# BAMresearch/PGDrome

Measured on AMD Instinct MI355X. Metric: PGD fixed-point iters/sec + SpMV HBM GB/s, 256^3 P1 space x 1D param, higher is better.
Workload: dtype f64

## Files before the change

include/pgd_amd.h:

```cpp
#ifndef PGD_AMD_H
#define PGD_AMD_H

#include <stdint.h>

#ifdef __cplusplus
extern "C" {
#endif

typedef int64_t pgd_handle;

enum {
    PGD_OK = 0,
    PGD_ERR_INVALID = -1,
    PGD_ERR_HIP = -2,
    PGD_ERR_NOMEM = -3,
    PGD_ERR_LIMIT = -4,
    PGD_ERR_SINGULAR = -5,
    PGD_ERR_NODEVICE = -6,
    PGD_ERR_TIMEOUT = -7,
    PGD_ERR_PEER = -8
};

enum {
    PGD_ATOM_MASS = 0,
// ... 9 lines not shown
};

int pgd_ctx_create(int device, void *stream, pgd_handle *ctx);
int pgd_ctx_destroy(pgd_handle ctx);
int pgd_sync(pgd_handle ctx);
const char *pgd_last_error(pgd_handle ctx);
int pgd_version(void);
int pgd_device_count(void);

int pgd_mesh_upload(pgd_handle ctx, const double *coords, int64_t nv, int gdim,
                    const int32_t *cells, int64_t nc, int nvpc, pgd_handle *mesh);
int pgd_mesh_blocked(pgd_handle ctx, pgd_handle scalar_mesh, int ncomp, pgd_handle *mesh);
int pgd_mesh_info(pgd_handle ctx, pgd_handle mesh, int64_t *nv, int64_t *nc, int64_t *nnz,
                  int32_t *max_row_len, int32_t *kl, int32_t *ku);
int pgd_mesh_pattern_download(pgd_handle ctx, pgd_handle mesh, int32_t *row_ptr, int32_t *cols);
int pgd_mesh_dict_count(pgd_handle ctx, pgd_handle mesh, int32_t *count);
int pgd_mesh_sym_info(pgd_handle ctx, pgd_handle mesh, int32_t *slots, int32_t *nx, int32_t *ny);
int pgd_mesh_lattice(pgd_handle ctx, pgd_handle mesh, int32_t *is_lattice, double *steps);
int pgd_mesh_free(pgd_handle ctx, pgd_handle mesh);

int pgd_vec_alloc(pgd_handle ctx, int64_t n, pgd_handle *vec);
int pgd_vec_free(pgd_handle ctx, pgd_handle vec);
int pgd_vec_size(pgd_handle ctx, pgd_handle vec, int64_t *n);
int pgd_vec_upload(pgd_handle ctx, pgd_handle vec, const double *host, int64_t offset, int64_t count);
int pgd_vec_download(pgd_handle ctx, pgd_handle vec, double *host, int64_t offset, int64_t count);
int pgd_vec_ptr(pgd_handle ctx, pgd_handle vec, void **device_ptr);
int pgd_vec_fill(pgd_handle ctx, pgd_handle vec, double value);
int pgd_vec_copy(pgd_handle ctx, pgd_handle dst, pgd_handle src);
int pgd_vec_scale(pgd_handle ctx, pgd_handle vec, double a);
int pgd_vec_mul(pgd_handle ctx, pgd_handle y, pgd_handle a, pgd_handle x);
int pgd_vec_axpy(pgd_handle ctx, pgd_handle y, double a, pgd_handle x);
int pgd_vec_set(pgd_handle ctx, pgd_handle vec, const int32_t *idx, const double *val, int64_t n);
int pgd_vec_lincomb(pgd_handle ctx, pgd_handle y, const pgd_handle *xs, const double *coefs, int k);
int pgd_vec_dot(pgd_handle ctx, pgd_handle x, pgd_handle y, int64_t lo, int64_t hi, double *out);

int pgd_atom_assemble(pgd_handle ctx, pgd_handle mesh, int kind, int da, int db,
                      pgd_handle wvec, pgd_handle *atom);
int pgd_atom_assemble_cells(pgd_handle ctx, pgd_handle mesh, int kind, int da, int db, pgd_handle wvec,
                            const uint8_t *cell_mask, int64_t nc, pgd_handle *atom);
int pgd_atom_assemble_cellwise(pgd_handle ctx, pgd_handle mesh, int kind, int da, int db, pgd_handle wvec,
                               pgd_handle cvec, const uint8_t *cell_mask, int64_t nc, pgd_handle *atom);
int pgd_atom_assemble_facets(pgd_handle ctx, pgd_handle mesh, const int32_t *facets, int64_t nf, int nvpf,
                             pgd_handle *atom);
int pgd_atom_embed(pgd_handle ctx, pgd_handle blocked_mesh, pgd_handle src, int cv, int cu, double coef,
                   pgd_handle dst, pgd_handle *out);
int pgd_atom_upload(pgd_handle ctx, pgd_handle mesh, const double *vals, pgd_handle *atom);
int pgd_atom_download(pgd_handle ctx, pgd_handle atom, double *vals);
int pgd_atom_free(pgd_handle ctx, pgd_handle atom);

int pgd_op_combine(pgd_handle ctx, pgd_handle mesh, const pgd_handle *atoms, const double *coefs,
                   int n, const int32_t *bc_dofs, int64_t nbc, pgd_handle *op);

int pgd_spmv(pgd_handle ctx, pgd_handle A, pgd_handle x, pgd_handle y, int64_t r0, int64_t r1);
int pgd_bilinear(pgd_handle ctx, pgd_handle A, pgd_handle x, pgd_handle y, int64_t r0, int64_t r1,
                 double *out);
int pgd_bilinear_many(pgd_handle ctx, pgd_handle A, pgd_handle x, const pgd_handle *ys, int ny,
                      int64_t r0, int64_t r1, double *out);

int pgd_pcg_solve(pgd_handle ctx, pgd_handle op, pgd_handle b, pgd_handle x, double rtol,
                  double atol, int maxit, int *iters, double *relres);
int pgd_band_solve(pgd_handle ctx, pgd_handle op, pgd_handle b, pgd_handle x);

#define PGD_NSLOTS 64
int pgd_slots_ptr(pgd_handle ctx, void **device_ptr);
int pgd_slots_download(pgd_handle ctx, double *out, int first, int count);
int pgd_slots_upload(pgd_handle ctx, const double *in, int first, int count);
// ... 39 lines not shown
                  int64_t hi_ghost);
int pgd_comm_allreduce_slots(pgd_handle ctx, int first_slot, int count);

#define PGD_PUSH_BLOB_BYTES 256
int pgd_comm_push_export(pgd_handle ctx, int64_t n, int64_t own0, int64_t own1, int64_t lo_ghost, int64_t hi_ghost,
                         uint8_t *blob );
int pgd_comm_push_attach(pgd_handle ctx, const uint8_t *lower_blob, const uint8_t *upper_blob, int *state);
int pgd_comm_push(pgd_handle ctx, int mode, int *state);
int pgd_comm_allreduce_attach(pgd_handle ctx, const uint8_t *all_blobs, int *state);
int pgd_comm_allreduce_direct(pgd_handle ctx, int mode, int *state);
int pgd_pcg_solve_sharded(pgd_handle ctx, pgd_handle A, pgd_handle b, pgd_handle x, int64_t own0,
                          int64_t own1, int64_t lo_ghost, int64_t hi_ghost, double rtol, double atol,
                          int maxit, int *iters, double *rel_res);

int pgd_bicgstab_solve(pgd_handle ctx, pgd_handle A, pgd_handle b, pgd_handle x, double rtol, double atol,
                       int maxit, int *iters, double *rel_res);

int pgd_start_gram(pgd_handle ctx, pgd_handle A, const pgd_handle *vecs, int k, pgd_handle b, int64_t r0,
                   int64_t r1, double *out);
int pgd_start_residual(pgd_handle ctx, pgd_handle A, int k, const double *coefs, pgd_handle b, pgd_handle r);

int pgd_vec_multidot(pgd_handle ctx, pgd_handle x, const pgd_handle *ys, int k, int64_t lo, int64_t hi,
                     double *out);

int pgd_vec_multidot_pair(pgd_handle ctx, pgd_handle x0, pgd_handle x1, const pgd_handle *ys, int k, int64_t lo,
                          int64_t hi, double *out);

enum { PGD_EVAL_STATS = 1, PGD_EVAL_ENVELOPE = 2, PGD_EVAL_EXCEED = 4, PGD_EVAL_FIELDS = 8 };
int pgd_eval_batch(pgd_handle ctx, const pgd_handle *modes, int k, const double *coefs, int64_t s, int want,
                   double threshold, double *sample_stats, pgd_handle env_min, pgd_handle env_max, pgd_handle exceed,
                   pgd_handle fields);

enum {
    PGD_TUNE_PCG_RECOMPUTE_Q = 53,
    PGD_TUNE_EVAL_SAMPLE_CHUNK = 52,
    PGD_TUNE_EVAL_GRID_MAX = 51,
    PGD_TUNE_EVAL_VARIANT = 50,
    PGD_TUNE_PUSH_IN_UPDATE = 49,
    PGD_TUNE_STENCIL_ROWS = 48,
    PGD_TUNE_DIA_MARCH3 = 47,
    PGD_TUNE_SHARD_ONE_MARCH = 46,
    PGD_TUNE_HALO_OVERLAP_MIN_ROWS = 45,
    PGD_TUNE_COMM_SELF_PERIODIC = 44,
    PGD_TUNE_PCG_DERIVE_SCALED = 43,
    PGD_TUNE_MG_MARCH_MIN = 42,
    PGD_TUNE_MG_CHUNK = 41,
    PGD_TUNE_PCG_PRECOND = 40,
    PGD_TUNE_CLS_CACHE = 39,
    PGD_TUNE_STENCIL_DEPTH = 38,
    PGD_TUNE_STENCIL_WG_PER_CU = 37,
    PGD_TUNE_SPMV_ZCHUNK_STENCIL = 36,
    PGD_TUNE_SPMV_STENCIL = 35,
    PGD_TUNE_FAULT_STALL_MS = 34,
    PGD_TUNE_FAULT_STAGE = 33,
    PGD_TUNE_SPMV_ZCHUNK_CODED2 = 32,
    PGD_TUNE_PCG_PIPELINE = 31,
    PGD_TUNE_PCG_EXACT_PHASE = 30,
    PGD_TUNE_PCG_FOLD_FINISH = 29,
    PGD_TUNE_LAZY_CSR = 28,
    PGD_TUNE_ATOM_FAST = 27,
    PGD_TUNE_SPMV_ROWS = 1,
    PGD_TUNE_SPMV_GRID_MIN_BYTES = 8,
    PGD_TUNE_PCG_FOLD_REDUCE = 12,
    PGD_TUNE_PCG_SCALED = 10,
    PGD_TUNE_SPMV_ZCHUNK_FORCE = 7,
    PGD_TUNE_PCG_SMALL_ROWS = 26,
// ... 49 lines not shown
```

pgdrome_amd/_lib.py:

```python
from __future__ import annotations

import ctypes as C
from pathlib import Path

import numpy as np

LIB_PATH = Path(__file__).resolve().parent / "lib" / "libpgd_amd.so"

H = C.c_int64
I64 = C.c_int64
I32 = C.c_int32
F64 = C.c_double
PD = C.POINTER(C.c_double)
PI32 = C.POINTER(C.c_int32)
PI64 = C.POINTER(C.c_int64)
PH = C.POINTER(C.c_int64)
VP = C.c_void_p

PU8 = C.POINTER(C.c_uint8)
HALO_FN = C.CFUNCTYPE(C.c_int, VP, H, I64, I64, I64, I64)
ALLREDUCE_FN = C.CFUNCTYPE(C.c_int, VP, C.c_int, C.c_int)

SIGNATURES = {
    "pgd_ctx_create": (C.c_int, [C.c_int, VP, PH]),
    "pgd_ctx_destroy": (C.c_int, [H]),
    "pgd_sync": (C.c_int, [H]),
    "pgd_last_error": (C.c_char_p, [H]),
    "pgd_version": (C.c_int, []),
    "pgd_device_count": (C.c_int, []),
    "pgd_mesh_upload": (C.c_int, [H, PD, I64, C.c_int, PI32, I64, C.c_int, PH]),
    "pgd_mesh_blocked": (C.c_int, [H, H, C.c_int, PH]),
    "pgd_atom_embed": (C.c_int, [H, H, H, C.c_int, C.c_int, F64, H, PH]),
    "pgd_mesh_info": (C.c_int, [H, H, PI64, PI64, PI64, PI32, PI32, PI32]),
    "pgd_mesh_pattern_download": (C.c_int, [H, H, PI32, PI32]),
    "pgd_mesh_sym_info": (C.c_int, [H, H, PI32, PI32, PI32]),
    "pgd_mesh_dict_count": (C.c_int, [H, H, PI32]),
    "pgd_mesh_lattice": (C.c_int, [H, H, PI32, PD]),
    "pgd_mesh_free": (C.c_int, [H, H]),
    "pgd_vec_alloc": (C.c_int, [H, I64, PH]),
    "pgd_vec_free": (C.c_int, [H, H]),
    "pgd_vec_size": (C.c_int, [H, H, PI64]),
    "pgd_vec_upload": (C.c_int, [H, H, PD, I64, I64]),
    "pgd_vec_download": (C.c_int, [H, H, PD, I64, I64]),
    "pgd_vec_ptr": (C.c_int, [H, H, C.POINTER(VP)]),
    "pgd_vec_fill": (C.c_int, [H, H, F64]),
    "pgd_vec_copy": (C.c_int, [H, H, H]),
    "pgd_vec_scale": (C.c_int, [H, H, F64]),
    "pgd_vec_mul": (C.c_int, [H, H, H, H]),
    "pgd_vec_axpy": (C.c_int, [H, H, F64, H]),
    "pgd_vec_set": (C.c_int, [H, H, PI32, PD, I64]),
    "pgd_vec_lincomb": (C.c_int, [H, H, PH, PD, C.c_int]),
    "pgd_vec_dot": (C.c_int, [H, H, H, I64, I64, PD]),
    "pgd_eval_batch": (C.c_int, [H, PH, C.c_int, PD, I64, C.c_int, F64, PD, H, H, H, H]),
    "pgd_atom_assemble": (C.c_int, [H, H, C.c_int, C.c_int, C.c_int, H, PH]),
    "pgd_atom_assemble_cells": (C.c_int, [H, H, C.c_int, C.c_int, C.c_int, H, PU8, I64, PH]),
    "pgd_atom_assemble_cellwise": (C.c_int, [H, H, C.c_int, C.c_int, C.c_int, H, H, PU8, I64, PH]),
    "pgd_atom_assemble_facets": (C.c_int, [H, H, PI32, I64, C.c_int, PH]),
    "pgd_atom_upload": (C.c_int, [H, H, PD, PH]),
    "pgd_atom_download": (C.c_int, [H, H, PD]),
    "pgd_atom_free": (C.c_int, [H, H]),
    "pgd_op_combine": (C.c_int, [H, H, PH, PD, C.c_int, PI32, I64, PH]),
    "pgd_spmv": (C.c_int, [H, H, H, H, I64, I64]),
    "pgd_bilinear": (C.c_int, [H, H, H, H, I64, I64, PD]),
    "pgd_bilinear_many": (C.c_int, [H, H, H, PH, C.c_int, I64, I64, PD]),
    "pgd_start_gram": (C.c_int, [H, H, PH, C.c_int, H, I64, I64, PD]),
    "pgd_start_residual": (C.c_int, [H, H, C.c_int, PD, H, H]),
    "pgd_mg_slab_setup": (C.c_int, [H, H, C.c_int, C.c_int, I64, I64, C.POINTER(I64), C.POINTER(C.c_int)]),
    "pgd_mg_slab_fix_start": (C.c_int, [H, H, H, H, I64, I64]),
    "pgd_mg_slab_down": (C.c_int, [H, H, H]),
    "pgd_mg_slab_restrict": (C.c_int, [H, H, H]),
    "pgd_mg_coarse": (C.c_int, [H, H, H]),
    "pgd_mg_slab_up": (C.c_int, [H, H, H, H, H, C.c_int, PD]),
    "pgd_bicgstab_solve": (C.c_int, [H, H, H, H, C.c_double, C.c_double, C.c_int, C.POINTER(C.c_int), PD]),
    "pgd_atom_product_form": (C.c_int, [H, H, C.POINTER(C.c_int)]),
    "pgd_vec_multidot": (C.c_int, [H, H, PH, C.c_int, I64, I64, PD]),
    "pgd_vec_multidot_pair": (C.c_int, [H, H, H, PH, C.c_int, I64, I64, PD]),
    "pgd_pcg_solve": (C.c_int, [H, H, H, H, F64, F64, C.c_int, C.POINTER(C.c_int), PD]),
    "pgd_band_solve": (C.c_int, [H, H, H, H]),
    "pgd_slots_ptr": (C.c_int, [H, C.POINTER(VP)]),
    "pgd_slots_download": (C.c_int, [H, PD, C.c_int, C.c_int]),
    "pgd_slots_upload": (C.c_int, [H, PD, C.c_int, C.c_int]),
    "pgd_flags_reset": (C.c_int, [H]),
    "pgd_flags_download": (C.c_int, [H, PI32, PI32, PI32]),
    "pgd_op_diag_inv": (C.c_int, [H, H, H]),
# ... 216 lines not shown
    def vec_download(self, v, offset=0, count=None):
        if count is None:
            count = self.vec_size(v) - offset
        out = np.empty(count, dtype=np.float64)
        self._ck(self.lib.pgd_vec_download(self.h, v, dptr(out), int(offset), int(count)))
        return out

    def vec_ptr(self, v):
        p = VP()
        self._ck(self.lib.pgd_vec_ptr(self.h, v, C.byref(p)))
        return p.value

    def vec_fill(self, v, a):
        self._ck(self.lib.pgd_vec_fill(self.h, v, float(a)))

    def vec_copy(self, dst, src):
        self._ck(self.lib.pgd_vec_copy(self.h, dst, src))

    def vec_scale(self, v, a):
        self._ck(self.lib.pgd_vec_scale(self.h, v, float(a)))

    def vec_mul(self, y, a, x):
        self._ck(self.lib.pgd_vec_mul(self.h, y, a, x))

    def vec_axpy(self, y, a, x):
        self._ck(self.lib.pgd_vec_axpy(self.h, y, float(a), x))

    def vec_lincomb(self, y, xs, coefs):
        k = len(xs)
        arr = (H * max(k, 1))(*[int(x) for x in xs])
        cf = np.ascontiguousarray(coefs, dtype=np.float64)
        self._ck(self.lib.pgd_vec_lincomb(self.h, y, arr, dptr(cf) if k else None, k))

    def eval_batch(self, modes, coefs, stats=True, env_min=0, env_max=0, exceed=0, threshold=0.0, fields=0):
        k = len(modes)
        cf = np.ascontiguousarray(coefs, dtype=np.float64)
        if cf.ndim != 2 or cf.shape[0] != k:
            raise ValueError("eval_batch: coefs must have shape (len(modes), samples), got %r for %d modes" % (cf.shape, k))
        s = cf.shape[1]
        want = (EVAL_STATS if stats else 0) | (EVAL_ENVELOPE if (env_min or env_max) else 0) | \
               (EVAL_EXCEED if exceed else 0) | (EVAL_FIELDS if fields else 0)
        arr = (H * max(k, 1))(*[int(x) for x in modes])
        out = np.empty((3, s), dtype=np.float64) if stats else None
        self._ck(self.lib.pgd_eval_batch(self.h, arr, k, dptr(cf) if cf.size else None, s, want, float(threshold),
                                         dptr(out) if stats else None, int(env_min), int(env_max), int(exceed), int(fields)))
        return out

    def vec_set(self, v, idx, val):
        idx = np.ascontiguousarray(idx, dtype=np.int32)
        val = np.ascontiguousarray(np.broadcast_to(np.asarray(val, dtype=np.float64), idx.shape))
        self._ck(self.lib.pgd_vec_set(self.h, v, iptr(idx), dptr(val), idx.size))

    def vec_dot(self, x, y, lo=0, hi=-1):
        out = F64()
        self._ck(self.lib.pgd_vec_dot(self.h, x, y, int(lo), int(hi), C.byref(out)))
        return out.value

    def vec_multidot(self, x, ys, lo=0, hi=-1):
        k = len(ys)
        arr = (H * k)(*[int(v) for v in ys])
        out = np.zeros(k, dtype=np.float64)
        self._ck(self.lib.pgd_vec_multidot(self.h, x, arr, k, int(lo), int(hi), dptr(out)))
        return out

    def vec_multidot_pair(self, x0, x1, ys, lo=0, hi=-1):
        k = len(ys)
# ... 395 lines not shown
```

pgdrome_amd/csrc/pgd_internal.h:

```cpp
#pragma once

#include <hip/hip_runtime.h>

#include <cstdint>
#include <cstdio>
#include <map>
#include <memory>
#include <string>
#include <vector>

#include "../../include/pgd_amd.h"

namespace pgd {

constexpr int WAVE = 64;
constexpr int TPB = 256;
constexpr int MAX_VEC_BLOCKS = 2048;
constexpr int N_XCD = 8;
constexpr int DICT_MAXP = 256;
constexpr int DICT_DLEN = 32;
constexpr size_t PAD_BYTES = 256;

enum { S_PQ = 2, S_TOL2 = 5, S_DMIN = 7 , S_TMP = 8  };
enum { S1_RZ = 24, S1_RR = 25, S1_ALPHA = 26, S1_BETA = 27, S1_PQ = 28, S1_QQ = 29,
// ... 161 lines not shown
    int *flags = nullptr;
    double *partials = nullptr;
    int64_t partials_cap = 0;
    int64_t partials_off = 0;
    double *work[7] = {nullptr, nullptr, nullptr, nullptr, nullptr, nullptr, nullptr};
    int64_t work_cap[7] = {0, 0, 0, 0, 0, 0, 0};
    uint8_t *mask = nullptr;
    int64_t mask_cap = 0;
    int *ibuf = nullptr;
    int64_t ibuf_cap = 0;
    std::vector<int32_t> set_idx_host;
    std::vector<double> set_val_host;
    int *set_idx = nullptr;
    double *set_vals = nullptr;
    int64_t set_idx_cap = 0, set_vals_cap = 0;
    int32_t set_idx_max = 0;
    bool set_idx_on_dev = false, set_val_on_dev = false;

    Comm comm;

    int num_cu = 256;
    int spmv_dict = 1;
    int spmv_rows = 64;
    int64_t spmv_grid_min_plane_bytes = 0;
    int spmv_zchunk_force = 0;
    int fault_iteration = -1;
    int fault_stage = 0;
    int fault_stall_ms = 0;
    int64_t pcg_small_ss_rows = (int64_t)1 << 22;
    int pcg_small_ss = 1;
    int pcg_stream_hints = 1;
    int pcg_lag_x = 1;
    int pcg_recompute_q = 1;
    int64_t pcg_recompute_launches = 0;
    int asm_lattice = 1;
    int spmv_fetch_depth = 6;
    int spmv_zchunk_coded2 = 96;
    int spmv_zchunk_coded = 24;
    int pcg_exact_phase = 1;
    int pcg_fold_finish = 1;
    int atom_fast = 1;
    int lazy_csr = 1;
    uint64_t next_serial = 1;
    int pcg_precond = 0;
    struct Mg *mg = nullptr;
    struct Mg *mg_slab = nullptr;
    int64_t mg_solves = 0, mg_fallbacks = 0;
    struct Vmg *vmg = nullptr;
    int64_t vmg_solves = 0, vmg_fallbacks = 0, vmg_marches = 0;
    double vmg_setup_ms = 0.0;
    struct Cmg *cmg = nullptr;
    int64_t cmg_solves = 0, cmg_fallbacks = 0, cmg_marches = 0;
    double cmg_setup_ms = 0.0;
    int eval_variant = 1, eval_grid_max = 0, eval_chunk = 0;
    double *eval_pin = nullptr;
    size_t eval_pin_bytes = 0;
    hipEvent_t eval_ev[2] = {nullptr, nullptr};
    bool eval_ev_set[2] = {false, false};
    int mg_chunk = 2;
    int mg_march_min = 64;
    int cls_cache_on = 1;
    int64_t cls_fast = 0, cls_full = 0;
    int spmv_stencil = 1;
    int spmv_zchunk_stencil = 0;
    int stencil_depth = 0;
    int stencil_wg_per_cu = 2;
// ... 213 lines not shown
```

pgdrome_amd/csrc/pgd_spmv.hip:

```cpp
#include <chrono>
#include <cstring>

#include "pgd_internal.h"
#include "pgd_dia_march.h"

#include <algorithm>

namespace pgd {

constexpr int SPMV_CAP = 4096;
constexpr int SPMV_VROUNDS = 8;
constexpr int SPMV_CROUNDS = 4;
constexpr int MAXY = 8;

struct SpmvArgs {
    const int *row_ptr, *cols;
    const double *vals, *x, *w;
    double *y, *partials;
    const int *flags;
    int row_begin, row_end;
};

typedef double d2_t __attribute__((ext_vector_type(2)));
typedef int i4_t __attribute__((ext_vector_type(4)));
// ... 2347 lines not shown
}

constexpr int GRAM_MAXV = 17;
struct MultiDotArgs {
    const double *w, *b;
    const double *v[GRAM_MAXV];
    int nv;
    int64_t lo, hi;
    double *partials;
};

__global__ __launch_bounds__(TPB) void k_multidot(MultiDotArgs A) {
    __shared__ double s_red[4];
    double acc[GRAM_MAXV + 1];
#pragma unroll
    for (int m = 0; m <= GRAM_MAXV; ++m) acc[m] = 0.0;
    for (int64_t i = A.lo + (int64_t)blockIdx.x * TPB + threadIdx.x; i < A.hi; i += (int64_t)gridDim.x * TPB) {
        const double wi = A.w[i];
        double last = 0.0;
#pragma unroll
        for (int m = 0; m < GRAM_MAXV; ++m)
            if (m < A.nv) { last = A.v[m][i]; acc[m] = fma(last, wi, acc[m]); }
        acc[GRAM_MAXV] = fma(last, A.b[i], acc[GRAM_MAXV]);
    }
#pragma unroll
    for (int m = 0; m <= GRAM_MAXV; ++m) {
        if (m < A.nv || m == GRAM_MAXV) {
            const double sum = block_sum(acc[m], s_red);
            if (threadIdx.x == 0) A.partials[(int64_t)blockIdx.x * (A.nv + 1) + (m == GRAM_MAXV ? A.nv : m)] = sum;
        }
    }
}

constexpr int PAIR_MAXV = 16;
struct MultiDot2Args {
    const double *w0, *w1;
    const double *v[PAIR_MAXV];
    int nv;
    int64_t lo, hi;
    double *partials;
};

__global__ __launch_bounds__(TPB) void k_multidot2(MultiDot2Args A) {
    __shared__ double s_red[4];
    double a0[PAIR_MAXV], a1[PAIR_MAXV];
#pragma unroll
    for (int m = 0; m < PAIR_MAXV; ++m) a0[m] = a1[m] = 0.0;
    for (int64_t i = A.lo + (int64_t)blockIdx.x * TPB + threadIdx.x; i < A.hi; i += (int64_t)gridDim.x * TPB) {
        const double x0 = A.w0[i], x1 = A.w1[i];
#pragma unroll
        for (int m = 0; m < PAIR_MAXV; ++m)
            if (m < A.nv) { const double y = A.v[m][i]; a0[m] = fma(y, x0, a0[m]); a1[m] = fma(y, x1, a1[m]); }
    }
#pragma unroll
    for (int m = 0; m < PAIR_MAXV; ++m) {
        if (m < A.nv) {
            const double s0 = block_sum(a0[m], s_red);
            const double s1 = block_sum(a1[m], s_red);
            if (threadIdx.x == 0) {
                A.partials[(int64_t)blockIdx.x * (2 * A.nv) + m] = s0;
                A.partials[(int64_t)blockIdx.x * (2 * A.nv) + A.nv + m] = s1;
            }
        }
    }
}

// ... 125 lines not shown
    if (knob == PGD_TUNE_STENCIL_WG_PER_CU && value >= 1 && value <= 8) { c->stencil_wg_per_cu = (int)value; return PGD_OK; }
    if (knob == PGD_TUNE_FAULT_STAGE && value >= 0 && value <= 4) { c->fault_stage = (int)value; return PGD_OK; }
    if (knob == PGD_TUNE_FAULT_STALL_MS && value >= 0 && value <= 20000) { c->fault_stall_ms = (int)value; return PGD_OK; }
    if (knob == PGD_TUNE_COMBINE_DIA && value >= 0 && value <= 1) { c->spmv_combine_dia = (int)value; return PGD_OK; }
    if (knob == PGD_TUNE_SPMV_VARIANT && value >= 0 && value <= 2) { c->spmv_variant = (int)value; return PGD_OK; }
    if (knob == PGD_TUNE_SPMV_ROW_CLASSES && value >= 0 && value <= 1) { c->spmv_classes = (int)value; return PGD_OK; }
    if (knob == PGD_TUNE_ASM_LATTICE && value >= 0 && value <= 3) { c->asm_lattice = (int)value; return PGD_OK; }
    if (knob == PGD_TUNE_PCG_LAG_X && value >= 0 && value <= 1) { c->pcg_lag_x = (int)value; return PGD_OK; }
    if (knob == PGD_TUNE_PCG_STREAM_HINTS && value >= 0 && value <= 1) { c->pcg_stream_hints = (int)value; return PGD_OK; }
    if (knob == PGD_TUNE_PCG_SMALL_SINGLE_SYNC && value >= 0 && value <= 1) { c->pcg_small_ss = (int)value; return PGD_OK; }
    if (knob == PGD_TUNE_PCG_SMALL_ROWS && value >= 0) { c->pcg_small_ss_rows = value; return PGD_OK; }
    if (knob == PGD_TUNE_SPMV_FETCH_DEPTH && (value == 3 || value == 6)) { c->spmv_fetch_depth = (int)value; return PGD_OK; }
    if (knob == PGD_TUNE_SPMV_ZCHUNK_CODED2 && value >= 0 && value <= 1020) { c->spmv_zchunk_coded2 = (int)value / 6 * 6; return PGD_OK; }
    if (knob == PGD_TUNE_PCG_PIPELINE && value >= 0 && value <= 1) { c->pcg_pipeline = (int)value; return PGD_OK; }
    if (knob == PGD_TUNE_PCG_EXACT_PHASE && value >= 0 && value <= 1) { c->pcg_exact_phase = (int)value; return PGD_OK; }
    if (knob == PGD_TUNE_PCG_FOLD_FINISH && value >= 0 && value <= 1) { c->pcg_fold_finish = (int)value; return PGD_OK; }
    if (knob == PGD_TUNE_ATOM_FAST && value >= 0 && value <= 1) { c->atom_fast = (int)value; return PGD_OK; }
    if (knob == PGD_TUNE_LAZY_CSR && value >= 0 && value <= 1) { c->lazy_csr = (int)value; return PGD_OK; }
    if (knob == PGD_TUNE_SPMV_ZCHUNK_CODED && value >= 3 && value <= 1024) { c->spmv_zchunk_coded = (int)value; return PGD_OK; }
    if (knob == PGD_TUNE_PCG_PRECOND && value >= 0 && value <= 3) { c->pcg_precond = (int)value; return PGD_OK; }
    if (knob == PGD_TUNE_PCG_DERIVE_SCALED && value >= 0 && value <= 1) { c->pcg_derive_scaled = (int)value; return PGD_OK; }
    if (knob == PGD_TUNE_COMM_SELF_PERIODIC && value >= 0 && value <= 1) { c->comm.self_periodic = value != 0; return PGD_OK; }
    if (knob == PGD_TUNE_HALO_OVERLAP_MIN_ROWS && value >= 0) { c->comm.overlap_min_rows = value; return PGD_OK; }
    if (knob == PGD_TUNE_SHARD_ONE_MARCH && value >= 0 && value <= 1) { c->shard_one_march = (int)value; return PGD_OK; }
    if (knob == PGD_TUNE_DIA_MARCH3 && value >= 0 && value <= 1) { c->dia_march3 = (int)value; return PGD_OK; }
    if (knob == PGD_TUNE_STENCIL_ROWS && (value == 0 || value == 2 || value == 4)) { c->stencil_rows = (int)value; return PGD_OK; }
    if (knob == PGD_TUNE_PUSH_IN_UPDATE && (value == 0 || value == 1)) { c->push_in_update = (int)value; return PGD_OK; }
    if (knob == PGD_TUNE_MG_CHUNK && value >= 2 && value <= 16 && value % 2 == 0) { c->mg_chunk = (int)value; return PGD_OK; }
    if (knob == PGD_TUNE_MG_MARCH_MIN && value >= 0 && value <= 1 << 20) { c->mg_march_min = (int)value; return PGD_OK; }
    if (knob == PGD_TUNE_EVAL_VARIANT && value >= 0 && value <= 1) { c->eval_variant = (int)value; return PGD_OK; }
    if (knob == PGD_TUNE_EVAL_GRID_MAX && value >= 0 && value <= 1 << 20) { c->eval_grid_max = (int)value; return PGD_OK; }
    if (knob == PGD_TUNE_EVAL_SAMPLE_CHUNK && value >= 0 && value <= 1024) { c->eval_chunk = (int)value; return PGD_OK; }
    if (knob == PGD_TUNE_PCG_RECOMPUTE_Q && value >= 0 && value <= 1) { c->pcg_recompute_q = (int)value; return PGD_OK; }
    return fail(c, PGD_ERR_INVALID, "tune: unknown knob %d or value out of range", knob);
}

int pgd_spmv(pgd_handle h, pgd_handle ah, pgd_handle xh, pgd_handle yh, int64_t r0, int64_t r1) {
    PGD_CTX(c, h);
    Csr *a = get_csr(c, ah);
    Mesh *m = a ? get_mesh(c, a->mesh) : nullptr;
    Vec *x = get_vec(c, xh), *y = get_vec(c, yh);
    if (!a || !m || !x || !y || x->n != m->nv || y->n != m->nv || x == y)
        return fail(c, PGD_ERR_INVALID, "spmv: invalid handles, size mismatch or x aliases y");
    if (atom_fast_form(c, m, a, r0, r1)) return launch_spmv_op(c, m, a, x->d, y->d, nullptr, r0, r1, false, true, nullptr, nullptr);
    if (c->spmv_sym && c->atom_fast && m->sym_nx > 0 && !a->immutable && a->uvals && a->uvals_valid && !a->uvals_scaled && !a->st_virtual) {
        const int64_t plane = (int64_t)m->sym_nx * m->sym_ny;
        const int64_t q0 = r0 < 0 ? 0 : r0, q1 = r1 < 0 ? m->nv : r1;
        if (q0 >= 0 && q1 <= m->nv && q0 <= q1 && q0 % plane == 0 && q1 % plane == 0)
            return launch_spmv_op(c, m, a, x->d, y->d, nullptr, q0, q1, false, true, nullptr, nullptr);
    }
    PGD_TRY(ensure_vals(c, m, a));
    return launch_spmv(c, m, a->vals, x->d, y->d, nullptr, r0, r1, false, true, nullptr, nullptr);
}

int pgd_bilinear(pgd_handle h, pgd_handle ah, pgd_handle xh, pgd_handle yh, int64_t r0, int64_t r1, double *out) {
    PGD_CTX(c, h);
    Csr *a = get_csr(c, ah);
    Mesh *m = a ? get_mesh(c, a->mesh) : nullptr;
    Vec *x = get_vec(c, xh), *y = get_vec(c, yh);
    if (!a || !m || !x || !y || !out || x->n != m->nv || y->n != m->nv)
        return fail(c, PGD_ERR_INVALID, "bilinear: invalid handles or size mismatch");
    int nparts = 0;
    PGD_TRY(ensure_vals(c, m, a));
    PGD_TRY(launch_spmv(c, m, a->vals, y->d, nullptr, x->d, r0, r1, true, false, nullptr, &nparts));
    if (nparts == 0) { *out = 0.0; return PGD_OK; }
    PGD_TRY(reduce_partials(c, c->partials, nparts, 1, S_TMP, -1, 0, 0));
// ... 58 lines not shown
    Csr *a = get_csr(c, ah);
    Mesh *m = a ? get_mesh(c, a->mesh) : nullptr;
    Vec *x = get_vec(c, xh), *y = get_vec(c, yh), *w = get_vec(c, wh);
    if (!a || !m || !x || !y || !w || x->n != m->nv || y->n != m->nv || w->n != m->nv || x == y ||
        slot < 0 || slot >= PGD_NSLOTS)
        return fail(c, PGD_ERR_INVALID, "spmv_dot_slot: invalid handles, sizes or slot");
    int nparts = 0;
    PGD_TRY(launch_spmv_op(c, m, a, x->d, y->d, w->d, r0, r1, true, true, c->flags, &nparts));
    if (nparts == 0) {
        PGD_HIP(c, hipMemsetAsync(c->slots + slot, 0, sizeof(double), c->stream));
        return PGD_OK;
    }
    return reduce_partials(c, c->partials, nparts, 1, slot, 0, 0, 0);
}

int pgd_vec_multidot(pgd_handle h, pgd_handle xh, const pgd_handle *yhs, int k, int64_t lo, int64_t hi, double *out) {
    PGD_CTX(c, h);
    Vec *x = get_vec(c, xh);
    if (!x || !yhs || !out || k < 1 || k > 256) return fail(c, PGD_ERR_INVALID, "vec_multidot: invalid handles or count (1..256)");
    if (hi < 0) hi = x->n;
    if (lo < 0 || lo > hi || hi > x->n) return fail(c, PGD_ERR_INVALID, "vec_multidot: bad range");
    std::vector<const double *> y((size_t)k);
    for (int j = 0; j < k; ++j) {
        Vec *v = get_vec(c, yhs[j]);
        if (!v || v->n != x->n) return fail(c, PGD_ERR_INVALID, "vec_multidot: invalid vector %d", j);
        y[(size_t)j] = v->d;
    }
    for (int j = 0; j < k; ++j) out[j] = 0.0;
    if (hi == lo) return PGD_OK;
    PGD_TRY(ensure_work(c, 6, 2 * (int64_t)MAX_VEC_BLOCKS > 512 ? 2 * (int64_t)MAX_VEC_BLOCKS : 512));
    double *res = c->work[6];
    const int g = grid_for(hi - lo);
    PGD_TRY(ensure_partials(c, (int64_t)g * (GRAM_MAXV + 1) > 4 * MAX_VEC_BLOCKS ? (int64_t)g * (GRAM_MAXV + 1) : 4 * MAX_VEC_BLOCKS));
    int off = 0;
    for (int j0 = 0; j0 < k; j0 += GRAM_MAXV) {
        const int nv = std::min(GRAM_MAXV, k - j0);
        MultiDotArgs A;
        A.w = x->d; A.b = x->d; A.nv = nv; A.lo = lo; A.hi = hi; A.partials = c->partials;
        for (int q = 0; q < GRAM_MAXV; ++q) A.v[q] = y[(size_t)(j0 + std::min(q, nv - 1))];
        k_multidot<<<g, TPB, 0, c->stream>>>(A);
        PGD_LAUNCH_CHECK(c);
        PGD_TRY(reduce_partials_to(c, c->partials, g, nv + 1, res + off));
        off += nv + 1;
    }
    std::vector<double> host((size_t)off);
    PGD_HIP(c, hipMemcpyAsync(host.data(), res, (size_t)off * sizeof(double), hipMemcpyDeviceToHost, c->stream));
    PGD_HIP(c, hipStreamSynchronize(c->stream));
    off = 0;
    for (int j0 = 0; j0 < k; j0 += GRAM_MAXV) {
        const int nv = std::min(GRAM_MAXV, k - j0);
        for (int q = 0; q < nv; ++q) out[j0 + q] = host[(size_t)(off + q)];
        off += nv + 1;
    }
    return PGD_OK;
}

int pgd_vec_multidot_pair(pgd_handle h, pgd_handle x0h, pgd_handle x1h, const pgd_handle *yhs, int k, int64_t lo, int64_t hi, double *out) {
    PGD_CTX(c, h);
    Vec *x0 = get_vec(c, x0h), *x1 = get_vec(c, x1h);
    if (!x0 || !x1 || x0->n != x1->n || !yhs || !out || k < 1 || k > 128)
        return fail(c, PGD_ERR_INVALID, "vec_multidot_pair: invalid handles or count (1..128)");
    if (hi < 0) hi = x0->n;
    if (lo < 0 || lo > hi || hi > x0->n) return fail(c, PGD_ERR_INVALID, "vec_multidot_pair: bad range");
    std::vector<const double *> y((size_t)k);
    for (int j = 0; j < k; ++j) {
        Vec *v = get_vec(c, yhs[j]);
// ... 121 lines not shown
```

pgdrome_amd/csrc/pgd_vec.hip:

```cpp
#include "pgd_internal.h"

#include <cstring>

namespace pgd {

__global__ __launch_bounds__(TPB) void k_fill(double *__restrict__ v, double a, int64_t n) {
    for (int64_t i = (int64_t)blockIdx.x * TPB + threadIdx.x; i < n; i += (int64_t)gridDim.x * TPB) v[i] = a;
}

__global__ __launch_bounds__(TPB) void k_scale(double *__restrict__ v, double a, int64_t n) {
    for (int64_t i = (int64_t)blockIdx.x * TPB + threadIdx.x; i < n; i += (int64_t)gridDim.x * TPB) v[i] *= a;
}

__global__ __launch_bounds__(TPB) void k_axpy(double *__restrict__ y, double a, const double *__restrict__ x, int64_t n) {
    for (int64_t i = (int64_t)blockIdx.x * TPB + threadIdx.x; i < n; i += (int64_t)gridDim.x * TPB)
        y[i] = fma(a, x[i], y[i]);
}

__global__ __launch_bounds__(TPB) void k_set(double *__restrict__ v, const int *__restrict__ idx,
                                             const double *__restrict__ val, int64_t n) {
    for (int64_t i = (int64_t)blockIdx.x * TPB + threadIdx.x; i < n; i += (int64_t)gridDim.x * TPB) v[idx[i]] = val[i];
}

struct LincombArgs {
    const double *x[8];
    double c[8];
    int k;
    int accumulate;
};

__global__ __launch_bounds__(TPB) void k_lincomb(double *__restrict__ y, LincombArgs A, int64_t n) {
    for (int64_t i = (int64_t)blockIdx.x * TPB + threadIdx.x; i < n; i += (int64_t)gridDim.x * TPB) {
        double s = A.accumulate ? y[i] : 0.0;
#pragma unroll
        for (int t = 0; t < 8; ++t)
            if (t < A.k) s = fma(A.c[t], A.x[t][i], s);
        y[i] = s;
    }
}

__global__ __launch_bounds__(TPB) void k_dot(const double *__restrict__ x, const double *__restrict__ y,
                                             int64_t lo, int64_t hi, double *__restrict__ partials) {
    __shared__ double s_red[4];
    double acc = 0.0;
    for (int64_t i = lo + (int64_t)blockIdx.x * TPB + threadIdx.x; i < hi; i += (int64_t)gridDim.x * TPB)
        acc = fma(x[i], y[i], acc);
    acc = block_sum(acc, s_red);
    if (threadIdx.x == 0) partials[blockIdx.x] = acc;
}

__global__ __launch_bounds__(1024) void k_reduce_partials(const double *__restrict__ partials, int nparts,
                                                          int nvals, double *__restrict__ slots, int slot0,
                                                          int check_mode, int slot_rr, int slot_tol2,
                                                          int *__restrict__ flags) {
    __shared__ double s_w[16];
    if (flags && check_mode >= 0 && flags[0]) return;
    const int lane = threadIdx.x & 63, wv = threadIdx.x >> 6;
    for (int v = 0; v < nvals; ++v) {
        double a8[8] = {0, 0, 0, 0, 0, 0, 0, 0};
        int i = threadIdx.x;
        for (; i + 7 * 1024 < nparts; i += 8 * 1024) {
#pragma unroll
            for (int u = 0; u < 8; ++u) a8[u] += partials[(int64_t)(i + u * 1024) * nvals + v];
        }
        for (int u = 0; i < nparts; i += 1024, ++u) a8[u & 7] += partials[(int64_t)i * nvals + v];
        double acc = ((a8[0] + a8[1]) + (a8[2] + a8[3])) + ((a8[4] + a8[5]) + (a8[6] + a8[7]));
        acc = wave_sum(acc);
        __syncthreads();
        if (lane == 0) s_w[wv] = acc;
        __syncthreads();
        if (threadIdx.x == 0) {
// ... 215 lines not shown
    if (!x || !y || !a || x->n != y->n || a->n != y->n) return fail(c, PGD_ERR_INVALID, "vec_mul: invalid handles or size mismatch");
    if (y->n == 0) return PGD_OK;
    k_vec_mul<<<grid_for(y->n), TPB, 0, c->stream>>>(y->d, a->d, x->d, y->n);
    PGD_LAUNCH_CHECK(c);
    return PGD_OK;
}

int pgd_vec_axpy(pgd_handle h, pgd_handle yh, double a, pgd_handle xh) {
    PGD_CTX(c, h);
    Vec *y = get_vec(c, yh), *x = get_vec(c, xh);
    if (!x || !y || x->n != y->n) return fail(c, PGD_ERR_INVALID, "vec_axpy: invalid handles or size mismatch");
    if (y->n == 0) return PGD_OK;
    k_axpy<<<grid_for(y->n), TPB, 0, c->stream>>>(y->d, a, x->d, y->n);
    PGD_LAUNCH_CHECK(c);
    return PGD_OK;
}

int pgd_vec_lincomb(pgd_handle h, pgd_handle yh, const pgd_handle *xs, const double *coefs, int k) {
    PGD_CTX(c, h);
    Vec *y = get_vec(c, yh);
    if (!y || k < 0 || (k > 0 && (!xs || !coefs))) return fail(c, PGD_ERR_INVALID, "vec_lincomb: bad arguments");
    std::vector<const double *> px((size_t)k);
    for (int t = 0; t < k; ++t) {
        Vec *x = get_vec(c, xs[t]);
        if (!x || x->n != y->n || x == y) return fail(c, PGD_ERR_INVALID, "vec_lincomb: vector %d invalid, of another size or aliasing y", t);
        px[t] = x->d;
    }
    if (y->n == 0) return PGD_OK;
    if (k == 0) {
        k_fill<<<grid_for(y->n), TPB, 0, c->stream>>>(y->d, 0.0, y->n);
        PGD_LAUNCH_CHECK(c);
        return PGD_OK;
    }
    for (int first = 0; first < k; first += 8) {
        LincombArgs A;
        A.k = (k - first < 8) ? k - first : 8;
        A.accumulate = first > 0;
        for (int t = 0; t < 8; ++t) { A.x[t] = px[first + (t < A.k ? t : 0)]; A.c[t] = (t < A.k) ? coefs[first + t] : 0.0; }
        k_lincomb<<<grid_for(y->n), TPB, 0, c->stream>>>(y->d, A, y->n);
    }
    PGD_LAUNCH_CHECK(c);
    return PGD_OK;
}

int pgd_start_residual(pgd_handle h, pgd_handle ah, int k, const double *coefs, pgd_handle bh, pgd_handle rh) {
    PGD_CTX(c, h);
    Vec *b = get_vec(c, bh), *r = get_vec(c, rh);
    if (!b || !r || b == r || !coefs || k < 1) return fail(c, PGD_ERR_INVALID, "start_residual: bad arguments");
    if (!c->gram_op || c->gram_op != ah || c->gram_k != k || c->gram_n != b->n || r->n != b->n || !c->gram_w)
        return fail(c, PGD_ERR_INVALID, "start_residual: the library does not hold the %d products of this operator "
                                        "(pgd_start_gram over all rows with at most 9 vectors must come right before)", k);
    int done = 0;
    bool first = true;
    while (done < k || first) {
        LincombArgs A;
        int t = 0;
        if (first) { A.x[0] = b->d; A.c[0] = 1.0; t = 1; }
        for (; t < 8 && done < k; ++t, ++done) { A.x[t] = c->gram_w + (size_t)done * (size_t)c->gram_n; A.c[t] = -coefs[done]; }
        A.k = t;
        A.accumulate = first ? 0 : 1;
        for (; t < 8; ++t) { A.x[t] = A.x[0]; A.c[t] = 0.0; }
        k_lincomb<<<grid_for(r->n), TPB, 0, c->stream>>>(r->d, A, r->n);
        first = false;
    }
    PGD_LAUNCH_CHECK(c);
    return PGD_OK;
}

int pgd_vec_set(pgd_handle h, pgd_handle vh, const int32_t *idx, const double *val, int64_t n) {
    PGD_CTX(c, h);
    Vec *v = get_vec(c, vh);
    if (!v || n < 0 || (n > 0 && (!idx || !val))) return fail(c, PGD_ERR_INVALID, "vec_set: bad arguments");
    if (n == 0) return PGD_OK;
    if (n < 4096) {
        for (int64_t i = 0; i < n; ++i)
            if (idx[i] < 0 || idx[i] >= v->n) return fail(c, PGD_ERR_INVALID, "vec_set: index %d out of range", idx[i]);
        PGD_TRY(ensure_ibuf(c, n));
        PGD_TRY(ensure_work(c, 5, n));
        PGD_HIP(c, hipMemcpyAsync(c->ibuf, idx, n * sizeof(int), hipMemcpyHostToDevice, c->stream));
        PGD_HIP(c, hipMemcpyAsync(c->work[5], val, n * sizeof(double), hipMemcpyHostToDevice, c->stream));
        k_set<<<grid_for(n), TPB, 0, c->stream>>>(v->d, c->ibuf, c->work[5], n);
        PGD_LAUNCH_CHECK(c);
        PGD_HIP(c, hipStreamSynchronize(c->stream));
        return PGD_OK;
// ... 79 lines not shown
```

pgdrome_amd/fem.py:

```python
from __future__ import annotations

import itertools
import logging
import math
import numbers
import os
import sys
import time
import weakref

import numpy as np

LOG = logging.getLogger("pgdrome_amd.fem")

MASS, STIFF, DUDV, CONV, CONVT, WMASS, WSTIFF = range(7)
WDUDV, WCONV, WCONVT = 7, 8, 9
_DA_KINDS, _DB_KINDS = (DUDV, CONV, WDUDV, WCONV), (DUDV, CONVT, WDUDV, WCONVT)
DS_MASS = "ds_mass"

_backend = None


def set_backend(be):
    global _backend
# ... 3192 lines not shown
        return v


SMALL_DIRECT_N = 20000
WARM_START_RESCALE = True
START_SPACE_MAX = int(os.environ.get("PGD_START_SPACE_MAX", "8"))


def _rescale_start(lay, op, b, x):
    be = get_backend()
    lo, hi = lay.owned_range()
    extras = [v for v in getattr(x, "_start_space", ()) if v is not x][-START_SPACE_MAX:]
    vecs = [x] + extras
    for v in vecs:
        _halo(lay, v)
    k = len(vecs)
    G, g = be.start_gram(op, [v.dev() for v in vecs], b.dev(), lo, hi)
    STATS["host_syncs_start"] = STATS.get("host_syncs_start", 0) + 1
    if lay.part is not None:
        packed = lay.part.comm.allreduce_array(np.concatenate([G.ravel(), g]))
        G, g = packed[:k * k].reshape(k, k), packed[k * k:]
    if not (np.all(np.isfinite(G)) and np.all(np.isfinite(g)) and G[0, 0] > 0.0):
        return None
    if k == 1:
        coef = np.array([g[0] / G[0, 0]])
    else:
        d = np.sqrt(np.abs(np.diag(G)))
        d[d == 0.0] = 1.0
        coef = np.linalg.lstsq(G / np.outer(d, d), g / d, rcond=1e-10)[0] / d
    if not np.all(np.isfinite(coef)) or not np.any(coef):
        return None
    if k == 1:
        be.vec_scale(x.dev(), float(coef[0]))
    else:
        out = be.vec_zeros(lay.n)
        be.vec_lincomb(out, [v.dev() for v in vecs], [float(c) for c in coef])
        be.vec_copy(x.dev(), out)
        be.vec_free(out)
    x.touched_dev()
    if lay.part is not None:
        x._halo_version = x.version
    return coef


def _solve_linear(A, b, x, prm):
    be, mesh = get_backend(), A.mesh()
    method = str(prm.get("linear_solver", "default"))
    n = A.lay.n
    op = A.op()
    info = {}
    part, view = A.lay.part, (A.lay.shard_view() if A.lay.part is not None else mesh)
    try:
        use_direct = mesh.topology().dim() == 1 and n <= SMALL_DIRECT_N and part is None
        nonsym = not use_direct and not A.is_symmetric()
        if use_direct:
            be.band_solve(op, b.dev(), x.dev_for_write())
            x.touched_dev()
            info.update(method="band_lu", iterations=1)
        elif nonsym:
            rtol = float(prm.get("relative_tolerance", 1e-10)) if not isinstance(prm.get("relative_tolerance"), _Params) else 1e-10
            atol = float(prm.get("absolute_tolerance", 0.0)) if not isinstance(prm.get("absolute_tolerance"), _Params) else 0.0
            maxit = int(prm.get("maximum_iterations", 20000)) if not isinstance(prm.get("maximum_iterations"), _Params) else 20000
            t_solve = time.perf_counter()
            if part is not None:
                it, rel = part.comm.bicgstab(view, op, b, x, rtol, atol, maxit)
            else:
# ... 205 lines not shown
```

pgdrome_amd/spectral.py:

```python
from __future__ import annotations

import logging
import os
import time
import weakref

import numpy as np

LOG = logging.getLogger("pgdrome_amd.spectral")
MIN_ROWS = int(os.environ.get("PGD_SPECTRAL_MIN_ROWS", "200000"))
RESIDUAL_BAR = 1e-2
STATS = {"harvests": 0, "harvest_seconds": 0.0, "corrections": 0, "dropped_requests": 0}
_SPACES = {}


GS_PASSES = int(os.environ.get("PGD_SPECTRAL_GS_PASSES", "2"))
AUTO_K = 32
AUTO_AFTER = 48
_AUTO_SOLVES = {}


def requested(prm):
    v = prm.get("spectral_start", None) if hasattr(prm, "get") else None
    if v is None or isinstance(v, dict):
# ... 41 lines not shown
    def correct(self, fem, A, op, b, x, start_coefs=None):
        be = fem.get_backend()
        lay = A.lay
        lo, hi = lay.owned_range()
        handles, coefs = A.merged()
        G = self.gram(fem, handles, coefs)
        if x._zero:
            r = b
        else:
            r = fem.Vector(b.V)
            held = False
            if start_coefs is not None and lay.part is None and hasattr(be, "start_residual"):
                try:
                    be.start_residual(op, start_coefs, b.dev(), r.dev_for_write())
                    held = True
                except Exception:
                    held = False
            if not held:
                fem._halo(lay, x)
                be.spmv(op, x.dev(), r.dev_for_write(), lo, hi)
                r.touched_dev()
                r.scale(-1.0)
                r.axpy(1.0, b)
            else:
                r.touched_dev()
        g = _multidot(fem, lay, r, self.Y)
        if not (np.all(np.isfinite(G)) and np.all(np.isfinite(g))):
            return False
        d = np.sqrt(np.abs(np.diag(G)))
        d[d == 0.0] = 1.0
        coef = np.linalg.lstsq(G / np.outer(d, d), g / d, rcond=1e-12)[0] / d
        if not np.all(np.isfinite(coef)) or not np.any(coef):
            return False
        out = be.vec_zeros(lay.n)
        vecs = [y.dev() for y in self.Y]
        cs = [float(c) for c in coef]
        if not x._zero:
            vecs, cs = [x.dev()] + vecs, [1.0] + cs
        be.vec_lincomb(out, vecs, cs)
        be.vec_copy(x.dev_for_write(), out)
        be.vec_free(out)
        x.touched_dev()
        if lay.part is not None:
            x._halo_version = -1
        STATS["corrections"] += 1
        return True


def _multidot(fem, lay, x, ys):
    be = fem.get_backend()
    lo, hi = lay.owned_range()
    out = []
    for i in range(0, len(ys), 16):
        chunk = ys[i:i + 16]
        v = be.vec_multidot(x.dev(), [y.dev() for y in chunk], lo, hi) if len(chunk) > 1 else [be.vec_dot(x.dev(), chunk[0].dev(), lo, hi)]
        out.extend(float(t) for t in v)
    out = np.array(out)
    if lay.part is not None:
        out = lay.part.comm.allreduce_array(out)
    return out


def _signature(A):
    bc = A.bc_vertices
    return (int(bc.size), hash(bc[:: max(1, bc.size // 4096)].tobytes()))


def get(fem, A, b, k, prm):
    key = (id(A.lay), _signature(A))
    hit = _SPACES.get(key, False)
    if hit is not False and (hit is None or hit.lay() is A.lay):
        return hit
    if k < 0:
        n = _AUTO_SOLVES.get(key, 0) + 1
        _AUTO_SOLVES[key] = n
        if n < AUTO_AFTER:
            return None
        k = -k
    sp = None
    try:
        sp = harvest(fem, A, b, k)
    except _Unavailable as e:
        STATS["dropped_requests"] += 1
        LOG.warning("spectral start asked for but not available on this system: %s", e)
    _SPACES[key] = sp
    if hit is False:
        weakref.finalize(A.lay, _SPACES.pop, key, None)
# ... 87 lines not shown
```

Baseline: 16.68.

## Add wide multidot and in-place lincomb kernels to cut vector passes

Adds templated wide kernels that handle up to 64 vectors per pass for multidot and linear combinations, replacing the 8/9-vector chunking that re-read x or y once per chunk. Adds an in-place lincomb_into entry point so callers scale and accumulate into x directly instead of allocating a temporary, combining and copying back. Python callers in fem and spectral now use it and batch multidot requests 256 vectors at a time. The trade-off is heavier register pressure from the large per-thread arrays, which may lower occupancy or cause spills.

```diff
diff --git a/include/pgd_amd.h b/include/pgd_amd.h
--- a/include/pgd_amd.h
+++ b/include/pgd_amd.h
@@ -65,6 +65,7 @@
 int pgd_vec_axpy(pgd_handle ctx, pgd_handle y, double a, pgd_handle x);
 int pgd_vec_set(pgd_handle ctx, pgd_handle vec, const int32_t *idx, const double *val, int64_t n);
 int pgd_vec_lincomb(pgd_handle ctx, pgd_handle y, const pgd_handle *xs, const double *coefs, int k);
+int pgd_vec_lincomb_into(pgd_handle ctx, pgd_handle y, double a, const pgd_handle *xs, const double *coefs, int k);
 int pgd_vec_dot(pgd_handle ctx, pgd_handle x, pgd_handle y, int64_t lo, int64_t hi, double *out);
 
 int pgd_atom_assemble(pgd_handle ctx, pgd_handle mesh, int kind, int da, int db,
@@ -170,6 +171,7 @@
                    pgd_handle fields);
 
 enum {
+    PGD_TUNE_VEC_WIDE = 54,
     PGD_TUNE_PCG_RECOMPUTE_Q = 53,
     PGD_TUNE_EVAL_SAMPLE_CHUNK = 52,
     PGD_TUNE_EVAL_GRID_MAX = 51,
diff --git a/pgdrome_amd/_lib.py b/pgdrome_amd/_lib.py
--- a/pgdrome_amd/_lib.py
+++ b/pgdrome_amd/_lib.py
@@ -50,6 +50,7 @@
     "pgd_vec_axpy": (C.c_int, [H, H, F64, H]),
     "pgd_vec_set": (C.c_int, [H, H, PI32, PD, I64]),
     "pgd_vec_lincomb": (C.c_int, [H, H, PH, PD, C.c_int]),
+    "pgd_vec_lincomb_into": (C.c_int, [H, H, C.c_double, PH, PD, C.c_int]),
     "pgd_vec_dot": (C.c_int, [H, H, H, I64, I64, PD]),
     "pgd_eval_batch": (C.c_int, [H, PH, C.c_int, PD, I64, C.c_int, F64, PD, H, H, H, H]),
     "pgd_atom_assemble": (C.c_int, [H, H, C.c_int, C.c_int, C.c_int, H, PH]),
@@ -332,6 +333,12 @@
         cf = np.ascontiguousarray(coefs, dtype=np.float64)
         self._ck(self.lib.pgd_vec_lincomb(self.h, y, arr, dptr(cf) if k else None, k))
 
+    def vec_lincomb_into(self, y, a, xs, coefs):
+        k = len(xs)
+        arr = (H * max(k, 1))(*[int(x) for x in xs])
+        cf = np.ascontiguousarray(coefs, dtype=np.float64)
+        self._ck(self.lib.pgd_vec_lincomb_into(self.h, y, float(a), arr, dptr(cf) if k else None, k))
+
     def eval_batch(self, modes, coefs, stats=True, env_min=0, env_max=0, exceed=0, threshold=0.0, fields=0):
         k = len(modes)
         cf = np.ascontiguousarray(coefs, dtype=np.float64)
diff --git a/pgdrome_amd/csrc/pgd_internal.h b/pgdrome_amd/csrc/pgd_internal.h
--- a/pgdrome_amd/csrc/pgd_internal.h
+++ b/pgdrome_amd/csrc/pgd_internal.h
@@ -217,6 +217,7 @@
     int pcg_stream_hints = 1;
     int pcg_lag_x = 1;
     int pcg_recompute_q = 1;
+    int vec_wide = 1;
     int64_t pcg_recompute_launches = 0;
     int asm_lattice = 1;
     int spmv_fetch_depth = 6;
diff --git a/pgdrome_amd/csrc/pgd_spmv.hip b/pgdrome_amd/csrc/pgd_spmv.hip
--- a/pgdrome_amd/csrc/pgd_spmv.hip
+++ b/pgdrome_amd/csrc/pgd_spmv.hip
@@ -2403,6 +2403,38 @@
     }
 }
 
+constexpr int MULTIDOT_WIDE = 64;
+struct MultiDotWideArgs {
+    const double *x;
+    const double *v[MULTIDOT_WIDE];
+    int nv;
+    int64_t lo, hi;
+    double *partials;
+};
+
+template <int NV>
+__global__ __launch_bounds__(TPB) void k_multidot_wide(MultiDotWideArgs A) {
+    __shared__ double s_red[4];
+    double acc[NV];
+#pragma unroll
+    for (int m = 0; m < NV; ++m) acc[m] = 0.0;
+    for (int64_t i = A.lo + (int64_t)blockIdx.x * TPB + threadIdx.x; i < A.hi; i += (int64_t)gridDim.x * TPB) {
+        double y[NV];
+#pragma unroll
+        for (int m = 0; m < NV; ++m) y[m] = A.v[m][i];
+        const double xi = A.x[i];
+#pragma unroll
+        for (int m = 0; m < NV; ++m) acc[m] = fma(y[m], xi, acc[m]);
+    }
+#pragma unroll
+    for (int m = 0; m < NV; ++m) {
+        if (m < A.nv) {
+            const double sum = block_sum(acc[m], s_red);
+            if (threadIdx.x == 0) A.partials[(int64_t)blockIdx.x * A.nv + m] = sum;
+        }
+    }
+}
+
 constexpr int PAIR_MAXV = 16;
 struct MultiDot2Args {
     const double *w0, *w1;
@@ -2594,6 +2626,7 @@
     if (knob == PGD_TUNE_EVAL_GRID_MAX && value >= 0 && value <= 1 << 20) { c->eval_grid_max = (int)value; return PGD_OK; }
     if (knob == PGD_TUNE_EVAL_SAMPLE_CHUNK && value >= 0 && value <= 1024) { c->eval_chunk = (int)value; return PGD_OK; }
     if (knob == PGD_TUNE_PCG_RECOMPUTE_Q && value >= 0 && value <= 1) { c->pcg_recompute_q = (int)value; return PGD_OK; }
+    if (knob == PGD_TUNE_VEC_WIDE && value >= 0 && value <= 1) { c->vec_wide = (int)value; return PGD_OK; }
     return fail(c, PGD_ERR_INVALID, "tune: unknown knob %d or value out of range", knob);
 }
 
@@ -2718,6 +2751,25 @@
     double *res = c->work[6];
     const int g = grid_for(hi - lo);
     PGD_TRY(ensure_partials(c, (int64_t)g * (GRAM_MAXV + 1) > 4 * MAX_VEC_BLOCKS ? (int64_t)g * (GRAM_MAXV + 1) : 4 * MAX_VEC_BLOCKS));
+    if (c->vec_wide) {
+        PGD_TRY(ensure_partials(c, std::max<int64_t>((int64_t)g * MULTIDOT_WIDE, 4 * MAX_VEC_BLOCKS)));
+        for (int j0 = 0; j0 < k; j0 += MULTIDOT_WIDE) {
+            const int nv = std::min(MULTIDOT_WIDE, k - j0);
+            MultiDotWideArgs A;
+            A.x = x->d; A.nv = nv; A.lo = lo; A.hi = hi; A.partials = c->partials;
+            for (int q = 0; q < MULTIDOT_WIDE; ++q) A.v[q] = y[(size_t)(j0 + std::min(q, nv - 1))];
+            if (nv <= 8) k_multidot_wide<8><<<g, TPB, 0, c->stream>>>(A);
+            else if (nv <= 16) k_multidot_wide<16><<<g, TPB, 0, c->stream>>>(A);
+            else if (nv <= 32) k_multidot_wide<32><<<g, TPB, 0, c->stream>>>(A);
+            else if (nv <= 48) k_multidot_wide<48><<<g, TPB, 0, c->stream>>>(A);
+            else k_multidot_wide<64><<<g, TPB, 0, c->stream>>>(A);
+            PGD_LAUNCH_CHECK(c);
+            PGD_TRY(reduce_partials_to(c, c->partials, g, nv, res + j0));
+        }
+        PGD_HIP(c, hipMemcpyAsync(out, res, (size_t)k * sizeof(double), hipMemcpyDeviceToHost, c->stream));
+        PGD_HIP(c, hipStreamSynchronize(c->stream));
+        return PGD_OK;
+    }
     int off = 0;
     for (int j0 = 0; j0 < k; j0 += GRAM_MAXV) {
         const int nv = std::min(GRAM_MAXV, k - j0);
diff --git a/pgdrome_amd/csrc/pgd_vec.hip b/pgdrome_amd/csrc/pgd_vec.hip
--- a/pgdrome_amd/csrc/pgd_vec.hip
+++ b/pgdrome_amd/csrc/pgd_vec.hip
@@ -1,5 +1,6 @@
 #include "pgd_internal.h"
 
+#include <algorithm>
 #include <cstring>
 
 namespace pgd {
@@ -37,6 +38,50 @@
             if (t < A.k) s = fma(A.c[t], A.x[t][i], s);
         y[i] = s;
     }
+}
+
+constexpr int LINCOMB_WIDE = 64;
+struct LincombWideArgs {
+    const double *x[LINCOMB_WIDE];
+    double c[LINCOMB_WIDE];
+    double a;
+    int k, start;
+};
+
+template <int NT>
+__global__ __launch_bounds__(TPB) void k_lincomb_wide(double *__restrict__ y, LincombWideArgs A, int64_t n) {
+    for (int64_t i = (int64_t)blockIdx.x * TPB + threadIdx.x; i < n; i += (int64_t)gridDim.x * TPB) {
+        double v[NT];
+#pragma unroll
+        for (int t = 0; t < NT; ++t) v[t] = A.x[t][i];
+        double s = A.start == 0 ? 0.0 : A.start == 1 ? y[i] : fma(A.a, y[i], 0.0);
+#pragma unroll
+        for (int t = 0; t < NT; ++t) {
+            const double st = fma(A.c[t], v[t], s);
+            s = t < A.k ? st : s;
+        }
+        y[i] = s;
+    }
+}
+
+int lincomb_wide(Ctx *c, double *y, int64_t n, const double *const *x, const double *cf, int nt, int start, double a) {
+    for (int first = 0; first < nt || first == 0; first += LINCOMB_WIDE) {
+        LincombWideArgs A;
+        A.k = std::min(LINCOMB_WIDE, nt - first);
+        A.start = first > 0 ? 1 : start;
+        A.a = a;
+        for (int t = 0; t < LINCOMB_WIDE; ++t) {
+            A.x[t] = t < A.k ? x[first + t] : (nt > 0 ? x[first] : y);
+            A.c[t] = t < A.k ? cf[first + t] : 0.0;
+        }
+        const int g = grid_for(n);
+        if (A.k <= 8) k_lincomb_wide<8><<<g, TPB, 0, c->stream>>>(y, A, n);
+        else if (A.k <= 16) k_lincomb_wide<16><<<g, TPB, 0, c->stream>>>(y, A, n);
+        else if (A.k <= 32) k_lincomb_wide<32><<<g, TPB, 0, c->stream>>>(y, A, n);
+        else k_lincomb_wide<64><<<g, TPB, 0, c->stream>>>(y, A, n);
+    }
+    PGD_LAUNCH_CHECK(c);
+    return PGD_OK;
 }
 
 __global__ __launch_bounds__(TPB) void k_dot(const double *__restrict__ x, const double *__restrict__ y,
@@ -318,6 +363,7 @@
         PGD_LAUNCH_CHECK(c);
         return PGD_OK;
     }
+    if (c->vec_wide) return lincomb_wide(c, y->d, y->n, px.data(), coefs, k, 0, 0.0);
     for (int first = 0; first < k; first += 8) {
         LincombArgs A;
         A.k = (k - first < 8) ? k - first : 8;
@@ -329,6 +375,41 @@
     return PGD_OK;
 }
 
+int pgd_vec_lincomb_into(pgd_handle h, pgd_handle yh, double a, const pgd_handle *xs, const double *coefs, int k) {
+    PGD_CTX(c, h);
+    Vec *y = get_vec(c, yh);
+    if (!y || k < 0 || (k > 0 && (!xs || !coefs))) return fail(c, PGD_ERR_INVALID, "vec_lincomb_into: bad arguments");
+    std::vector<const double *> px((size_t)k);
+    for (int t = 0; t < k; ++t) {
+        Vec *x = get_vec(c, xs[t]);
+        if (!x || x->n != y->n || x == y) return fail(c, PGD_ERR_INVALID, "vec_lincomb_into: vector %d invalid, of another size or aliasing y", t);
+        px[t] = x->d;
+    }
+    if (y->n == 0) return PGD_OK;
+    if (c->vec_wide) return lincomb_wide(c, y->d, y->n, px.data(), coefs, k, 2, a);
+    const size_t bytes = (size_t)y->n * sizeof(double);
+    void *pt;
+    PGD_TRY(dev_alloc(c, &pt, bytes));
+    double *tmp = (double *)pt;
+    hipError_t e = hipMemsetAsync(tmp, 0, bytes, c->stream);
+    for (int first = 0; first < k + 1 && e == hipSuccess; first += 8) {
+        LincombArgs A;
+        A.k = (k + 1 - first < 8) ? k + 1 - first : 8;
+        A.accumulate = first > 0;
+        for (int t = 0; t < 8; ++t) {
+            const int j = first + (t < A.k ? t : 0);
+            A.x[t] = j == 0 ? y->d : px[(size_t)j - 1];
+            A.c[t] = t < A.k ? (j == 0 ? a : coefs[j - 1]) : 0.0;
+        }
+        k_lincomb<<<grid_for(y->n), TPB, 0, c->stream>>>(tmp, A, y->n);
+    }
+    if (e == hipSuccess) e = hipMemcpyAsync(y->d, tmp, bytes, hipMemcpyDeviceToDevice, c->stream);
+    dev_release(c, tmp, bytes);
+    if (e != hipSuccess) return fail(c, PGD_ERR_HIP, "vec_lincomb_into: %s", hipGetErrorString(e));
+    PGD_LAUNCH_CHECK(c);
+    return PGD_OK;
+}
+
 int pgd_start_residual(pgd_handle h, pgd_handle ah, int k, const double *coefs, pgd_handle bh, pgd_handle rh) {
     PGD_CTX(c, h);
     Vec *b = get_vec(c, bh), *r = get_vec(c, rh);
@@ -336,6 +417,13 @@
     if (!c->gram_op || c->gram_op != ah || c->gram_k != k || c->gram_n != b->n || r->n != b->n || !c->gram_w)
         return fail(c, PGD_ERR_INVALID, "start_residual: the library does not hold the %d products of this operator "
                                         "(pgd_start_gram over all rows with at most 9 vectors must come right before)", k);
+    if (c->vec_wide && k < LINCOMB_WIDE) {
+        const double *px[LINCOMB_WIDE];
+        double cf[LINCOMB_WIDE];
+        px[0] = b->d; cf[0] = 1.0;
+        for (int j = 0; j < k; ++j) { px[j + 1] = c->gram_w + (size_t)j * (size_t)c->gram_n; cf[j + 1] = -coefs[j]; }
+        return lincomb_wide(c, r->d, r->n, px, cf, k + 1, 0, 0.0);
+    }
     int done = 0;
     bool first = true;
     while (done < k || first) {
diff --git a/pgdrome_amd/fem.py b/pgdrome_amd/fem.py
--- a/pgdrome_amd/fem.py
+++ b/pgdrome_amd/fem.py
@@ -3248,6 +3248,8 @@
         return None
     if k == 1:
         be.vec_scale(x.dev(), float(coef[0]))
+    elif hasattr(be, "vec_lincomb_into"):
+        be.vec_lincomb_into(x.dev(), float(coef[0]), [v.dev() for v in extras], [float(c) for c in coef[1:]])
     else:
         out = be.vec_zeros(lay.n)
         be.vec_lincomb(out, [v.dev() for v in vecs], [float(c) for c in coef])
diff --git a/pgdrome_amd/spectral.py b/pgdrome_amd/spectral.py
--- a/pgdrome_amd/spectral.py
+++ b/pgdrome_amd/spectral.py
@@ -97,14 +97,17 @@
         coef = np.linalg.lstsq(G / np.outer(d, d), g / d, rcond=1e-12)[0] / d
         if not np.all(np.isfinite(coef)) or not np.any(coef):
             return False
-        out = be.vec_zeros(lay.n)
         vecs = [y.dev() for y in self.Y]
         cs = [float(c) for c in coef]
-        if not x._zero:
-            vecs, cs = [x.dev()] + vecs, [1.0] + cs
-        be.vec_lincomb(out, vecs, cs)
-        be.vec_copy(x.dev_for_write(), out)
-        be.vec_free(out)
+        if x._zero:
+            be.vec_lincomb(x.dev_for_write(), vecs, cs)
+        elif hasattr(be, "vec_lincomb_into"):
+            be.vec_lincomb_into(x.dev(), 1.0, vecs, cs)
+        else:
+            out = be.vec_zeros(lay.n)
+            be.vec_lincomb(out, [x.dev()] + vecs, [1.0] + cs)
+            be.vec_copy(x.dev_for_write(), out)
+            be.vec_free(out)
         x.touched_dev()
         if lay.part is not None:
             x._halo_version = -1
@@ -116,8 +119,8 @@
     be = fem.get_backend()
     lo, hi = lay.owned_range()
     out = []
-    for i in range(0, len(ys), 16):
-        chunk = ys[i:i + 16]
+    for i in range(0, len(ys), 256):
+        chunk = ys[i:i + 256]
         v = be.vec_multidot(x.dev(), [y.dev() for y in chunk], lo, hi) if len(chunk) > 1 else [be.vec_dot(x.dev(), chunk[0].dev(), lo, hi)]
         out.extend(float(t) for t in v)
     out = np.array(out)
```

New measurement: 16.63. About the same (-0.3%).
